# WithSecureOpenSource/async

Measured on AMD Instinct MI355X. Metric: GiB/s base64 encode+decode, device-resident, at 1/2/4/8 MI355X, higher is better.
Workload: dtype u8; 1 GPU; cfg2: one 1 GiB buffer per GPU, encode (std alphabet, pad) then decode, device-resident; bytes_per_gpu=1073741824, chars_per_gpu=1431655768, parallelism=independent buffers x1 (no data-path collective)

## Files before the change

### async_amd/_lib.py

```python
from __future__ import annotations

import ctypes
import errno
import os
import threading

_HERE = os.path.dirname(os.path.abspath(__file__))
LIB_PATH = os.path.join(_HERE, "libasync_b64.so")

_lock = threading.Lock()
_lib = None


class B64xError(RuntimeError):

    def __init__(self, func: str, code: int):
        self.code = code
        name = errno.errorcode.get(-code, str(code))
        super().__init__(f"{func} failed: {name} ({code})")


class Alphabet(ctypes.Structure):

    _fields_ = [
# ... 48 lines not shown
    "b64x_session_host_out": (_vp, [_vp]),
    "b64x_session_encode": (_int, [_vp, _u64, _ap, ctypes.POINTER(_u64)]),
    "b64x_release_stream": (None, [_vp]),
    "b64x_session_decode": (_int, [_vp, _u64, _ap, ctypes.c_uint, ctypes.POINTER(DecResult)]),
    "b64x_session_encode_async": (_int, [_vp, _u64, _ap, _vp, _vp]),
    "b64x_session_decode_async": (_int, [_vp, _u64, _ap, ctypes.c_uint, _vp, _vp]),
    "b64x_session_result": (ctypes.POINTER(DecResult), [_vp]),
    "b64x_session_decode_result": (_int, [_vp, ctypes.POINTER(DecResult)]),
    "b64x_session_wait": (_int, [_vp]),
    "b64x_host_alloc": (_vp, [_u64]),
    "b64x_host_free": (None, [_vp]),
    "b64x_lane_open": (_vp, []),
    "b64x_lane_close": (None, [_vp]),
    "b64x_lane_acquire": (_vp, []),
    "b64x_lane_release": (None, [_vp]),
    "b64x_lane_encode_async": (_int, [_vp, _vp, _u32, _vp, _vp, _vp, _vp, _u32, _ap, _vp, _vp]),
    "b64x_lane_encode_check": (_int, [_vp]),
    "b64x_lane_decode_async": (_int, [_vp, _vp, _u32, _vp, _vp, _vp, _vp, _vp, _vp, _vp, _ap,
                                      _vp, _vp, ctypes.POINTER(_u32)]),
    "b64x_lane_decode_check": (_int, [_vp, _u32, _vp, _vp, _vp, _vp, _vp, _u32]),
    "b64x_lane_wait": (_int, [_vp]),
    "b64x_diag_counters": (None, [ctypes.POINTER(_u64)]),
    "b64x_diag_paths": (None, [ctypes.POINTER(_u64)]),
    "b64x_fill_splitmix64": (_int, [_vp, _u64, _u64, _vp]),
    "b64x_device_check": (_int, []),
    "b64x_device_numa_node": (_int, [_int]),
    "b64x_bind_thread": (_int, [_int]),
    "b64x_build_info": (ctypes.c_char_p, []),
    "b64x_strerror": (ctypes.c_char_p, [_int]),
}

STAGE_SYMBOLS = [
    "base64_encode", "base64encoder_as_bytestream_1", "base64encoder_read",
    "base64encoder_close", "base64encoder_register_callback",
    "base64encoder_unregister_callback",
    "base64_decode", "base64decoder_as_bytestream_1", "base64decoder_read",
    "base64decoder_close", "base64decoder_register_callback",
    "base64decoder_unregister_callback",
    "make_async", "destroy_async", "async_now", "async_timer_start",
    "async_timer_cancel", "async_execute", "async_wound", "async_loop",
    "async_quit_loop", "async_register", "async_unregister",
    "NULL_ACTION_1", "bytestream_1_close_relaxed",
    "open_blobstream", "copy_blobstream", "adopt_blobstream",
    "blobstream_as_bytestream_1", "blobstream_remaining", "blobstream_read",
    "blobstream_close", "blobstream_register_callback",
    "blobstream_unregister_callback",
    "make_nice", "nicestream_as_bytestream_1", "nicestream_read",
    "nicestream_close", "nicestream_register_callback",
    "nicestream_unregister_callback",
]


def _import_torch_first() -> None:
    try:
        import torch
    except ImportError:
        pass


_DIAG_ONLY = {"b64x_diag_paths"}


def load() -> ctypes.CDLL:
    global _lib
    with _lock:
        if _lib is not None:
            return _lib
        if not os.path.exists(LIB_PATH):
            raise RuntimeError(
                f"{LIB_PATH} is missing: build it with `make` or "
                "__graft_entry__.build(); there is no CPU fallback")
        _import_torch_first()
        lib = ctypes.CDLL(LIB_PATH)
        for name, (res, args) in SIGNATURES.items():
            if name in _DIAG_ONLY and not hasattr(lib, name):
                continue
            fn = getattr(lib, name)
            fn.restype = res
            fn.argtypes = args
        _lib = lib
        return lib


# ... 18 lines not shown
```

### async_amd/csrc/b64x_kernels.hip

```cpp
#include <hip/hip_runtime.h>

#include <errno.h>
#include <sched.h>
#include <stdint.h>
#include <stdio.h>
#include <stdlib.h>
#include <string.h>
#include <sys/syscall.h>
#include <unistd.h>

#include <atomic>
#include <mutex>
#include <type_traits>
#include <utility>

#include "b64x.h"
#include "b64x_result_check.h"

#define DEV __device__ __forceinline__

namespace {

constexpr int kThreads = 256;
constexpr int kWavesPerBlock = kThreads / 64;
// ... 1395 lines not shown
    const uint32_t t2 = tab[(x >> 16) & 0xFFu], t3 = tab[x >> 24];
    const uint32_t lo = __builtin_amdgcn_perm(t1, t0, 0x0c0c0400u);
    const uint32_t hi = __builtin_amdgcn_perm(t3, t2, 0x0c0c0400u);
    return __builtin_amdgcn_perm(hi, lo, 0x05040100u);
}

constexpr uint32_t kProbeThreads = 256;

struct DecodeHint {
    uint32_t key, junky;
};
constexpr uint32_t kDecodeHints = 64;
constexpr uint64_t kProbeSampleMin = 1u << 18;
constexpr uint32_t kProbeNS = 256;
constexpr uint64_t kProbeTailKeep = 4096;

struct ProbeSmem {
    uint8_t tab[256];
    LineModel m;
    unsigned long long first;
};

DEV void probe_stream(ProbeSmem &ps, const uint8_t *__restrict__ in, uint64_t n, DecAlpha a,
                      void *ws, uint32_t nranges, DecodeHint *hint, uint32_t key, uint32_t publish)
{
    uint8_t *const tab = ps.tab;
    LineModel &s_m = ps.m;
    unsigned long long &s_first = ps.first;
    const bool sample = n >= kProbeSampleMin && threadIdx.x < kProbeNS;
    uint32_t sw[16];
    uint64_t q = 0;
    if (sample) {
        const uint64_t W = n - kProbeTailKeep - 64 - 256;
        const uint64_t span = threadIdx.x < kProbeNS / 2 ? W / 16 : W;
        const uint64_t i = threadIdx.x % (kProbeNS / 2) + 1;
        const uint64_t raw = 256 + span * i * i / ((uint64_t) kProbeNS * kProbeNS / 4);
        const uint8_t *pa = (const uint8_t *) ((uintptr_t) (in + raw) & ~(uintptr_t) 15);
        q = (uint64_t) (pa - in);
#pragma unroll
        for (uint32_t k = 0; k < 4; k++) {
            const uint4 x = *(const uint4 *) (pa + 16 * k);
            sw[4 * k] = x.x;
            sw[4 * k + 1] = x.y;
            sw[4 * k + 2] = x.z;
            sw[4 * k + 3] = x.w;
        }
    }
// ... 33 lines not shown
            const bool want = m.L == 0 || r < m.L;
            if (al != want && first == ~0ull) first = q + j;
            if (m.L && ++r == m.P) r = 0;
        }
        if (first != ~0ull) atomicMin(&s_first, (unsigned long long) first);
    }
    block_sync();
    if (threadIdx.x != 0) return;
    LineModel mo = m;
    const uint64_t pf = s_first;
    if (!mo.skip && pf != ~0ull) {
        const uint64_t F = mo.L ? pf / mo.P * mo.L + (pf % mo.P < mo.L ? pf % mo.P : mo.L) : pf;
        if (F / 16 < mo.T) {
            mo.T = (uint32_t) (F / 16);
            mo.skip = 1;
        }
    }
    if (mo.skip && publish) {
        *ws_view(ws, nranges).lfail = ~(uint64_t) mo.T;
        *ws_view(ws, nranges).fail_any = 1;
    }
    *ws_view(ws, nranges).model = mo;
    *ws_view(ws, nranges).model_n = n;
    if (hint) {
        volatile DecodeHint *h = hint;
        h->junky = mo.skip && 256 * (uint64_t) mo.T < n ? 1u : 0u;
        h->key = key;
    }
}

__global__ void __launch_bounds__(kProbeThreads) k_decode_probe(const uint8_t *__restrict__ in, uint64_t n,
                                                                DecAlpha a, void *ws, uint32_t nranges,
                                                                DecodeHint *hint, uint32_t key)
{
    __shared__ ProbeSmem ps;
    probe_stream(ps, in, n, a, ws, nranges, hint, key, 1u);
}

constexpr uint32_t kLinesTH = 256, kLinesWaves = kLinesTH / 64;

DEV void lines_first_fail(uint32_t badm, uint32_t &fail_u, uint32_t &fail_lane)
{
    if (__ballot(badm != 0) == 0) return;
#pragma unroll
    for (uint32_t u = 0; u < kLinesU; u++) {
        const uint64_t fb = __ballot((badm >> u) & 1u);
        if (fb) {
            fail_u = u;
            fail_lane = (uint32_t) __ffsll((unsigned long long) fb) - 1;
            return;
        }
    }
}

template <bool A4>
DEV uint32_t lines_hot(const uint8_t *tab, const uint8_t *__restrict__ inw, uint32_t pos0,
                       uint8_t *__restrict__ outw, uint32_t obase, const LineModel &m,
                       uint32_t col0, uint32_t lane)
{
// ... 13 lines not shown
        oo[u] = pos & 3u;
        const uint8_t *ab = inw + (pos & ~3u);
        win[u] = ld16<false>(ab);
        const u32x2a4 v = *(const u32x2a4 *) (ab + 16);
        wx[u] = make_uint2(v.x, v.y);
    }
    const uint32_t need = sep_need(s);
    uint32_t badm = 0;
#pragma unroll
    for (uint32_t u = 0; u < kLinesU; u++) {
        const uint32_t w6[6] = {win[u].x, win[u].y, win[u].z, win[u].w, wx[u].x, wx[u].y};
        uint32_t sep, G[4], bad;
        const uint4 d = A4 ? slot_chars4(w6, oo[u], cc[u] >> 2, s, &sep)
                           : slot_chars(w6, oo[u], cc[u], s, &sep);
        map_fast(tab, d, 16, G, bad);
        const uint32_t nd = hs[u] ? need : 0u;
        if ((sep_nonalpha(tab, sep) & nd) != nd) bad |= 0x100u;
        badm |= bad ? 1u << u : 0u;
        emit_full_off<true>(G, outw, obase + 12 * (u * 64 + lane));
    }
    return badm;
}

template <bool BIG>
__global__ __launch_bounds__(kLinesTH) __attribute__((amdgpu_waves_per_eu(6)))
void k_decode_lines(
    const uint8_t *__restrict__ in, uint64_t n, uint8_t *__restrict__ out, uint32_t nranges,
    DecAlpha a, void *ws, uint32_t hold, b64x_dec_result *res, uint32_t seq)
{
    __shared__ uint8_t tab[256];
    __shared__ uint8_t s_tail[64];
    const uint64_t *mp = (const uint64_t *) ws_view(ws, nranges).model;
    const uint64_t mw0 = scalar_load_u64(mp), mw1 = scalar_load_u64(mp + 1),
                   mw2 = scalar_load_u64(mp + 2), mw3 = scalar_load_u64(mp + 3);
    const uint64_t mn = scalar_load_u64(ws_view(ws, nranges).model_n);
    build_dec_table(tab, a);
    const bool mok = mn == n;
    const uint32_t T = mok ? (uint32_t) (mw1 >> 32) : (uint32_t) (n / 16);
    if (blockIdx.x * kLinesWaves * kLinesSlots > T) return;
    block_sync();
    LineModel m;
    m.L = mok ? (uint32_t) mw0 : 0u;
    m.s = (uint32_t) (mw0 >> 32);
    m.P = (uint32_t) mw1;
    m.T = T;
    m.m = (uint32_t) mw2;
    m.k = (uint32_t) (mw2 >> 32);
    m.rcp = (uint32_t) mw3;
    m.skip = mok ? (uint32_t) (mw3 >> 32) : 0u;
    const uint32_t lane = lane_id();
    const uint32_t L = m.L, s = m.s, P = m.P;
    const uint32_t wv = (uint32_t) __builtin_amdgcn_readfirstlane((int) (threadIdx.x >> 6));
    const uint32_t t0 = (blockIdx.x * kLinesWaves + wv) * kLinesSlots;
    if (t0 > T) return;
    const uint32_t ns = T - t0 >= kLinesSlots ? kLinesSlots : T - t0;
    const bool full = ns == kLinesSlots;
    const bool oal = (((uintptr_t) out) & 3) == 0;
    const bool ial = (((uintptr_t) in) & 3) == 0;
    uint32_t fail_u = kLinesU, fail_lane = 0;
    const uint64_t i0 = 16ull * t0;
    const uint32_t line0 = !L ? 0u : !BIG ? line_div(m, (uint32_t) i0) : (uint32_t) (i0 / L);
    const uint32_t col0 = (uint32_t) (i0 - (uint64_t) line0 * L);
    const uint64_t ie = i0 + 16 * ns;
    const uint32_t le = !L ? 0u : !BIG ? line_div(m, (uint32_t) ie) : (uint32_t) (ie / L);
    const bool safe = (L ? (uint64_t) le * P + (ie - (uint64_t) le * L) : ie) + 24 <= n;
    const uint64_t pos0 = (uint64_t) line0 * P;
    uint8_t *const outw = BIG ? out + 12ull * t0 : out;
    const uint32_t obase = BIG ? 0u : 12 * t0;
    if (ns && L == 0 && full && oal && ial) {
        uint4 c[kLinesU];
        const uint8_t *const inw = BIG ? in + 16ull * t0 : in;
        const uint32_t ibase = BIG ? 0u : 16 * t0;
#pragma unroll
        for (uint32_t u = 0; u < kLinesU; u++) c[u] = ld16<true>(inw + (ibase + 16 * (u * 64 + lane)));
        uint32_t badm = 0;
#pragma unroll
        for (uint32_t u = 0; u < kLinesU; u++) {
            uint32_t G[4], bad;
            map_fast(tab, c[u], 16, G, bad);
            badm |= bad ? 1u << u : 0u;
            emit_full_off<true>(G, outw, obase + 12 * (u * 64 + lane));
        }
        lines_first_fail(badm, fail_u, fail_lane);
    } else if (ns && L != 0 && full && oal && ial && safe) {
        const uint8_t *const inw = BIG ? in + (pos0 & ~3ull) : in;
        const uint32_t p0 = (uint32_t) (BIG ? pos0 & 3u : pos0);
        const uint32_t badm = (L & 3) == 0
            ? lines_hot<true>(tab, inw, p0, outw, obase, m, col0, lane)
            : lines_hot<false>(tab, inw, p0, outw, obase, m, col0, lane);
        lines_first_fail(badm, fail_u, fail_lane);
    } else if (ns) {
        uint32_t G[kLinesU][4], bad[kLinesU];
        const uint8_t *end = in + n;
        uint4 win[kLinesU];
        uint2 wx[kLinesU];
        uint32_t oo[kLinesU], cc[kLinesU];
        bool hs[kLinesU];
#pragma unroll
        for (uint32_t u = 0; u < kLinesU; u++) {
            const uint32_t rel = col0 + 16 * (u * 64 + lane);
            const uint32_t dl = L ? (rel * m.rcp) >> 20 : 0;
            const uint32_t col = rel - dl * L;
            const uint64_t pos = L ? (uint64_t) (line0 + dl) * P + col : i0 + 16 * (u * 64 + lane);
            hs[u] = L && L - col <= 16;
            cc[u] = hs[u] ? L - col : 16u;
            const uint8_t *ap = in + pos;
            const uint8_t *ab = (const uint8_t *) ((uintptr_t) ap & ~(uintptr_t) 3);
            oo[u] = (uint32_t) (ap - ab);
            const bool live = u * 64 + lane < ns;
            win[u] = live ? load_win16(ab, end) : make_uint4(0, 0, 0, 0);
            wx[u] = live ? load_win8(ab + 16, end) : make_uint2(0, 0);
        }
#pragma unroll
        for (uint32_t u = 0; u < kLinesU; u++) {
            const uint32_t w6[6] = {win[u].x, win[u].y, win[u].z, win[u].w, wx[u].x, wx[u].y};
            uint32_t sep;
            const uint4 d = slot_chars(w6, oo[u], cc[u], s, &sep);
            map_fast(tab, d, 16, G[u], bad[u]);
            const uint32_t need = sep_need(s);
            if (hs[u] && (sep_nonalpha(tab, sep) & need) != need) bad[u] |= 0x100u;
        }
#pragma unroll
        for (uint32_t u = 0; u < kLinesU; u++) {
            const bool live = u * 64 + lane < ns;
            const uint64_t fb = __ballot(live && bad[u] != 0);
            if (fb && fail_u == kLinesU) {
                fail_u = u;
                fail_lane = (uint32_t) __ffsll((unsigned long long) fb) - 1;
            }
            if (live) {
                uint32_t o0, o1, o2;
                groups_to_bytes(G[u][0], G[u][1], G[u][2], G[u][3], o0, o1, o2);
                store_bytes12(out + 12 * (uint64_t) (t0 + u * 64 + lane), o0, o1, o2, 12);
            }
        }
    }
    const bool cut = m.skip && T < t0 + kLinesSlots;
    if ((fail_u < kLinesU || cut) && lane == 0) {
        const unsigned long long key =
            ~(unsigned long long) (fail_u < kLinesU ? t0 + fail_u * 64 + fail_lane : T);
        unsigned long long *lf = (unsigned long long *) ws_view(ws, nranges).lfail +
                                 (blockIdx.x % kFailWords) * kFailStride;
        const unsigned long long cur =
            __hip_atomic_load(lf, __ATOMIC_RELAXED, __HIP_MEMORY_SCOPE_AGENT);
        if (key > cur) atomicMax(lf, key);
        if (cur == 0) *ws_view(ws, nranges).fail_any = 1;
    }
    if (T >= t0 + kLinesSlots || m.skip) return;
    const uint64_t Q = line_pos(m, 16 * (uint64_t) T);
    const uint32_t tl = (uint32_t) (n - Q);
    const bool here = lane < tl;
    const uint32_t tv = here ? tab[in[Q + lane]] : 0xFFu;
    const bool al = tv < 64u;
    const uint64_t mb = __ballot(al);
    const uint32_t Vt = (uint32_t) __popcll(mb);
    const uint32_t rank = __builtin_amdgcn_mbcnt_hi((uint32_t) (mb >> 32),
                                                    __builtin_amdgcn_mbcnt_lo((uint32_t) mb, 0u));
    if (al) s_tail[rank] = (uint8_t) tv;
    wave_lds_order();
// ... 3 lines not shown
        const uint32_t G = ((uint32_t) s_tail[4 * lane] << 18) | ((uint32_t) s_tail[4 * lane + 1] << 12) |
                           ((uint32_t) s_tail[4 * lane + 2] << 6) | s_tail[4 * lane + 3];
        ot[3 * lane] = (uint8_t) (G >> 16);
        ot[3 * lane + 1] = (uint8_t) (G >> 8);
        ot[3 * lane + 2] = (uint8_t) G;
    } else if (lane == ng && !hold && rem >= 2) {
        const uint32_t G = ((uint32_t) s_tail[4 * ng] << 18) | ((uint32_t) s_tail[4 * ng + 1] << 12) |
                           (rem > 2 ? (uint32_t) s_tail[4 * ng + 2] << 6 : 0u);
        ot[3 * ng] = (uint8_t) (G >> 16);
        if (rem > 2) ot[3 * ng + 1] = (uint8_t) (G >> 8);
    }
    if (lane == 0) {
        const uint64_t V = 16 * (uint64_t) T + Vt;
        b64x_dec_result r;
        r.out_len = hold ? V / 4 * 3 : V * 6 / 8;
        r.valid = V;
        r.tail_n = rem;
        for (uint32_t j = 0; j < 4; j++) r.tail[j] = j < rem ? s_tail[4 * ng + j] : 0;
        r.nchars = n;
        r.seq = seq;
        r.flags = hold ? 1u : 0u;
        *res = r;
    }
}

DEV void decode_range(const P2dSmem &sm, uint4 *bq, const uint8_t *__restrict__ in, uint64_t n,
                      uint64_t start, uint64_t re, int T0, uint8_t *ob, const uint4 c[2],
                      const uint32_t nin[2], uint32_t la, bool la_ok, bool last, uint32_t hold,
                      const uint8_t *la_lds = nullptr, bool la_late = false)
{
    const uint32_t lane = lane_id();
    uint32_t *bits = (uint32_t *) bq;
    int T = T0;
    const uint32_t skew = (uint32_t) ((uintptr_t) ob & 15);
    uint32_t lo = 16 + skew;
    int pb0 = 8 * (int) lo;
    uint32_t done = 0;
    static_assert(kP2dBlocks > 64 && kP2dBlocks <= 128, "two zeroing stores per lane");
    bq[lane] = make_uint4(0, 0, 0, 0);
    if (lane + 64 < kP2dBlocks) bq[lane + 64] = make_uint4(0, 0, 0, 0);
    wave_lds_order();
    T += (int) bits_step<true>(sm, bits, c, nin, pb0 + 6 * T);
    for (uint64_t pos = start + 2 * kChunk; pos < re; pos += 2 * kChunk) {
        wave_lds_order();
        const int bit_end = pb0 + 6 * T;
        const uint32_t kcut = bit_end > 0 ? ((uint32_t) bit_end >> 3) & ~15u : 0u;
// ... 131 lines not shown
        uint64_t B = scalar_load_u64(w.bases + r);
        while (r < mid_end) {
            const uint32_t rn = r + nw < mid_end ? r + nw : r;
            uint4 cn[2];
            cn[0] = load16_a4(in + (uint64_t) rn * R + 16 * lane);
            cn[1] = load16_a4(in + (uint64_t) rn * R + kChunk + 16 * lane);
            const uint32_t lan = ld_la(rn);
            const uint64_t Bn = scalar_load_u64(w.bases + rn);
            const uint64_t rb = (uint64_t) r * R;
            decode_range(sm, bq, in, n, rb, rb + R, range_skip(B), out + (B + 3) / 4 * 3, c, full,
                         la, (uint64_t) (r + 1) * R + lane < n, false, hold);
            r += nw;
            c[0] = cn[0];
            c[1] = cn[1];
            la = lan;
            B = Bn;
        }
    }
    for (; r < nranges; r += nw) generic(r);
}


DEV bool suffix_start(DecodeWs w, uint64_t n, b64x_dec_result *res, b64x_dec_result *hres,
                      uint64_t &S, uint64_t &Vb, uint32_t *reprobe)
{
    __shared__ uint64_t s_key;
    uint64_t key = 0;
    if (scalar_load_u64(w.fail_any) != 0) {
        if (threadIdx.x < 64) {
            key = __hip_atomic_load((unsigned long long *) w.lfail + (threadIdx.x % kFailWords) *
                                    kFailStride, __ATOMIC_RELAXED, __HIP_MEMORY_SCOPE_AGENT);
#pragma unroll
            for (int d = 32; d >= 1; d >>= 1) {
                const uint64_t o = __shfl_xor(key, d, 64);
                key = o > key ? o : key;
            }
        }
        if (threadIdx.x == 0) s_key = key;
        block_sync();
        key = s_key;
    }
    if (key == 0) {
        if (blockIdx.x == 0 && threadIdx.x == 0) {
            if (hres) {
                const b64x_dec_result r = *res;
                *hres = r;
            }
            *w.sfx_start = ~0ull;
        }
        return false;
    }
    Vb = 16 * ~key;
    S = scalar_load_u64(w.model_n) == n ? line_pos(*w.model, Vb) : Vb;
    if (reprobe && blockIdx.x == 0 && threadIdx.x == 0) *(volatile uint32_t *) reprobe = 1u;
    return true;
}


DEV uint32_t window_delta(uint32_t s, const uint8_t *dst)
{
    const uint32_t a = (uint32_t) ((uintptr_t) dst & 15);
    const uint32_t i0 = (s + (a ? 128u : 0u) - 8 * a) >> 5;
    return (4u - (i0 & 3u)) & 3u;
}

typedef uint32_t v4u32 __attribute__((ext_vector_type(4)));
typedef __attribute__((address_space(3))) const v4u32 lds_v4u32;

DEV void store_window_bits(const uint32_t *win, uint32_t s, uint32_t nb, uint8_t *dst)
{
    const uint32_t lane = lane_id();
    s = (uint32_t) __builtin_amdgcn_readfirstlane((int) s);
    nb = (uint32_t) __builtin_amdgcn_readfirstlane((int) nb);
    const uint32_t a = (uint32_t) ((uintptr_t) dst & 15);
    const uint32_t m0 = a ? 1u : 0u, mend = (nb + a) >> 4;
    const uint32_t b0 = s + 128 * m0 - 8 * a;
// ... 14 lines not shown
        const v4u32 g4 = __builtin_nontemporal_load((const lds_v4u32 *) (win + i));
        const uint4 g = make_uint4(g4.x, g4.y, g4.z, g4.w);
        const uint32_t w4 = win[i + 4];
        uint32_t o0 = g.x, o1 = g.y, o2 = g.z, o3 = g.w;
        if (sh) {
            const uint32_t r = 32u - sh;
            o0 = __builtin_amdgcn_alignbit(g.x, g.y, r);
            o1 = __builtin_amdgcn_alignbit(g.y, g.z, r);
            o2 = __builtin_amdgcn_alignbit(g.z, g.w, r);
            o3 = __builtin_amdgcn_alignbit(g.w, w4, r);
        }
        if (k < nblk)
            __builtin_nontemporal_store(u32x4a16{bswap32(o0), bswap32(o1), bswap32(o2), bswap32(o3)},
                                        (u32x4a16 *) (base + 16 * k));
    }
    if (act) dst[bi] = (uint8_t) ((((uint64_t) x0 << 32) | x1) >> (56 - (X & 31)));
}

template <bool WHOLE, bool BIG>
__global__ __launch_bounds__(kThreads) __attribute__((amdgpu_waves_per_eu(kHeldWaves)))
void k_decode_suffix_held(
    const uint8_t *__restrict__ in, uint64_t n, uint8_t *__restrict__ out, uint32_t nranges,
    DecAlpha a, void *ws, uint32_t hold, b64x_dec_result *res, b64x_dec_result *hres,
    uint32_t seq, uint32_t *reprobe, DecodeHint *hint, uint32_t key)
{
    constexpr uint64_t R = 2 * kChunk;
    constexpr uint32_t HP = kHeldPer, TILE = kHeldTile;
    DecodeWs w = ws_view(ws, nranges);
    uint64_t S = 0, Vb = 0;
    if (!WHOLE && !suffix_start(w, n, res, hres, S, Vb, reprobe)) return;
    uint8_t *base_out = out + Vb / 4 * 3;
    const uint32_t r0 = (uint32_t) (S / R);
    const uint32_t ntiles = (nranges - r0 + TILE - 1) / TILE;
    if (!WHOLE && blockIdx.x == 0 && threadIdx.x == 0) *w.sfx_start = S;
    const bool dma = (((uintptr_t) in) & 15) == 0;
    __shared__ P2dSmem sm;
    __shared__ uint4 s_rng[kWavesPerBlock][2][128];
    __shared__ uint32_t s_tile[2];
    using Cnt = typename std::conditional<BIG, uint64_t, uint32_t>::type;
    __shared__ uint32_t s_cnt[2][TILE];
    __shared__ Cnt s_excl;
    build_dec_table_lo(sm.tab, a);
    build_compact_sel<true>(sm.sel);
    const uint32_t lane = lane_id();
    const uint32_t wv = __builtin_amdgcn_readfirstlane(threadIdx.x >> 6);
    uint4 *bq = sm.bits[wv];
    uint32_t *bits = (uint32_t *) bq;

    auto publish = [&](uint32_t t, uint32_t b) {
        uint32_t agg = 0;
        for (uint32_t i = 0; i < TILE; i++) agg += s_cnt[b][i];
        st_store(&w.fstatus[t], kStAgg | agg);
        __hip_atomic_fetch_add(&w.fsuper[t / kSfxGroup], (1ull << 56) | agg, __ATOMIC_RELAXED,
// ... 179 lines not shown
                }
            }
            if (tA == ntiles - 1) {
                owner = true;
                Vs = exw;
                for (uint32_t i = 0; i < TILE; i++) Vs += s_cnt[bA][i];
            }
        }
        if (!haveB) break;
        LA = LB;
#pragma unroll
        for (uint32_t j = 0; j < HP; j++) {
#pragma unroll
            for (int i = 0; i < 6; i++) HA[j][i] = HB[j][i];
        }
        haveA = true;
        tA = tB;
        bA = bB;
        bB ^= 1u;
        if (threadIdx.x == 0) s_tile[bB] = atomicAdd(w.fticket, 1u);
    }
    if (WHOLE && hint && s_tile[bB] == ntiles) {
        __shared__ ProbeSmem ps;
        probe_stream(ps, in, n, a, ws, nranges, hint, key, 0u);
    }
    block_sync();
    if (threadIdx.x == 0) __hip_atomic_fetch_add(w.wdone, 1u, __ATOMIC_RELAXED, __HIP_MEMORY_SCOPE_AGENT);
    if (!owner || wv != 0) return;
    const uint64_t V = Vb + Vs;
    if (lane == 0) write_result(res, hres, V, hold, n, seq);
    find_tail_sextets<true>(sm.tab, in, n, V, res, hres);
    if (lane == 0) {
        while (__hip_atomic_load(w.wdone, __ATOMIC_RELAXED, __HIP_MEMORY_SCOPE_AGENT) != gridDim.x)
            __builtin_amdgcn_s_sleep(1);
    }
    for (uint32_t i = lane; i < ntiles; i += 64) st_store(&w.fstatus[i], 0);
    for (uint32_t i = lane; i < (ntiles + kSfxGroup - 1) / kSfxGroup; i += 64) st_store(&w.fsuper[i], 0);
    if (lane == 0) {
        __hip_atomic_store(w.fticket, 0u, __ATOMIC_RELAXED, __HIP_MEMORY_SCOPE_AGENT);
        __hip_atomic_store(w.wdone, 0u, __ATOMIC_RELAXED, __HIP_MEMORY_SCOPE_AGENT);
        for (uint32_t i = 0; i < kFailWords; i++) w.lfail[i * kFailStride] = 0;
        *w.fail_any = 0;
    }
}

struct BatchLayout {
    const uint64_t *in_off;
// ... 1379 lines not shown

struct HeldModel {
    const void *ws;
    uint64_t n;
};
constexpr int kHeldModels = 64;
std::mutex g_held_mu;
HeldModel g_held[kHeldModels];

static uint32_t *held_reprobe(int slot)
{
    static uint32_t *h = nullptr;
    static std::once_flag once;
    std::call_once(once, [] {
        void *p = nullptr;
        if (hipHostMalloc(&p, kHeldModels * 64, hipHostMallocCoherent) == hipSuccess) {
            memset(p, 0, kHeldModels * 64);
            h = (uint32_t *) p;
        }
    });
    return h ? h + 16 * slot : nullptr;
}

static int held_slot(const void *ws)
{
    const uint64_t x = (uintptr_t) ws * 0x9E3779B97F4A7C15ull;
    return (int) (x >> 58);
}

enum { kPathProbe, kPathHeld, kPathHinted, kPathRowsPrep, kPathRowsReuse, kPaths };
static std::atomic<uint64_t> g_paths[kPaths];

static void path_taken(int k) { g_paths[k].fetch_add(1, std::memory_order_relaxed); }

void b64x_diag_paths(uint64_t out[5])
{
    for (int k = 0; k < kPaths; k++) out[k] = g_paths[k].load(std::memory_order_relaxed);
}

static uint32_t hint_key(const void *ws, const void *in, uint64_t n)
{
    uint64_t x = (uintptr_t) ws * 0x9E3779B97F4A7C15ull ^ (uintptr_t) in * 0xC2B2AE3D27D4EB4Full ^
                 n * 0x165667B19E3779F9ull;
    x ^= x >> 31;
    return (uint32_t) (x >> 32) | 1u;
}


static int decode_dev_ws(const void *d_in, uint64_t nchars, void *d_out,
                         b64x_dec_result *d_res, b64x_dec_result *h_res,
                         const b64x_alphabet *abc, unsigned flags, void *ws, void *stream,
                         uint32_t seq, const DeviceInfo *d)
{
    hipStream_t s = (hipStream_t) stream;
    int err = 0;
    const RangePlan p = plan_ranges(nchars);
    const uint32_t blocks = (p.nranges + kWavesPerBlock - 1) / kWavesPerBlock;
    const DecAlpha a = dec_alpha(abc);
    const uint32_t hold = flags & B64X_DEC_HOLD_TAIL;
    if (p.R == 2 * kChunk) {
        const bool big = nchars > (1ull << 31);
        static const int occ_small = occupancy_of(k_decode_suffix_held<false, false>);
        static const int occ_big = occupancy_of(k_decode_suffix_held<false, true>);
        const int occ_sfx = big ? occ_big : occ_small;
        auto *const k_whole = big ? k_decode_suffix_held<true, true> : k_decode_suffix_held<true, false>;
        auto *const k_sfx = big ? k_decode_suffix_held<false, true> : k_decode_suffix_held<false, false>;
        auto *const k_lines = big ? k_decode_lines<true> : k_decode_lines<false>;
        const uint32_t sfx_grid = (uint32_t) d->cus * occ_sfx;
        if (flags & B64X_DEC_EXPECT_JUNK) {
            hipLaunchKernelGGL(k_whole, dim3(sfx_grid), dim3(kThreads), 0, s,
                               (const uint8_t *) d_in, nchars, (uint8_t *) d_out, p.nranges, a, ws,
                               hold, d_res, h_res, seq, nullptr, nullptr, 0u);
            return launch_status();
        }
        DecodeHint *hints = decode_hints();
        const uint32_t key = hint_key(ws, d_in, nchars);
        DecodeHint *hint = hints ? hints + (key % kDecodeHints) : nullptr;
        const bool junky = hint && ((volatile DecodeHint *) hint)->key == key &&
                           ((volatile DecodeHint *) hint)->junky;
        const int hs = held_slot(ws);
        uint32_t *reprobe = held_reprobe(hs);
        bool reuse = false;
        if (!junky && reprobe && !capturing(stream)) {
            std::lock_guard<std::mutex> lk(g_held_mu);
            reuse = g_held[hs].ws == ws && g_held[hs].n == nchars &&
                    !*(volatile uint32_t *) reprobe;
        }
        if (junky) {
            path_taken(kPathHinted);
            if (reprobe) *(volatile uint32_t *) reprobe = 0;
            hipLaunchKernelGGL(k_whole, dim3(sfx_grid), dim3(kThreads), 0, s,
                               (const uint8_t *) d_in, nchars, (uint8_t *) d_out, p.nranges, a, ws,
                               hold, d_res, h_res, seq, nullptr, hint, key);
            if ((err = launch_status())) return err;
            path_taken(kPathProbe);
            std::lock_guard<std::mutex> lk(g_held_mu);
            g_held[hs] = HeldModel{ws, nchars};
            return 0;
        }
        if (!reuse) {
            if (reprobe) *(volatile uint32_t *) reprobe = 0;
            hipLaunchKernelGGL(k_decode_probe, dim3(1), dim3(kProbeThreads), 0, s,
                               (const uint8_t *) d_in, nchars, a, ws, p.nranges, hint, key);
            if ((err = launch_status())) return err;
            path_taken(kPathProbe);
            std::lock_guard<std::mutex> lk(g_held_mu);
            g_held[hs] = HeldModel{ws, nchars};
        } else {
            path_taken(kPathHeld);
        }
        const uint64_t waves = (nchars / 16 + 1 + kLinesSlots - 1) / kLinesSlots;
        hipLaunchKernelGGL(k_lines, dim3((uint32_t) ((waves + kLinesWaves - 1) / kLinesWaves)),
                           dim3(kLinesTH), 0, s, (const uint8_t *) d_in, nchars, (uint8_t *) d_out,
                           p.nranges, a, ws, hold, d_res, seq);
        if ((err = launch_status())) return err;
        hipLaunchKernelGGL(k_sfx, dim3(sfx_grid), dim3(kThreads), 0, s,
                           (const uint8_t *) d_in, nchars, (uint8_t *) d_out, p.nranges, a, ws,
                           hold, d_res, h_res, seq, reprobe, nullptr, 0u);
        return launch_status();
    }
    hipLaunchKernelGGL(k_pass1, dim3(blocks), dim3(kThreads), 0, s, (const uint8_t *) d_in,
                       nchars, (uint8_t *) d_out, p.R, p.nranges, a, ws, hold);
    if ((err = launch_status())) return err;
    hipLaunchKernelGGL(k_decode_scan2, dim3((p.nranges + kScanTile - 1) / kScanTile),
                       dim3(kThreads), 0, s, (const uint8_t *) d_in, nchars, p.R, p.nranges, a,
                       ws, d_res, h_res, hold, seq);
    if ((err = launch_status())) return err;
    static const int occ2d = occupancy_of(k_decode_pass2d);
    const uint32_t b2 = cap_grid(blocks, (uint64_t) d->cus * occ2d);
    hipLaunchKernelGGL(k_decode_pass2d, dim3(b2), dim3(kThreads), 0, s,
                       (const uint8_t *) d_in, nchars, (uint8_t *) d_out, p.R, p.nranges,
                       a, ws, hold);
    return launch_status();
}

static int decode_dev_impl(const void *d_in, uint64_t nchars, void *d_out,
                           b64x_dec_result *d_res, b64x_dec_result *h_res,
                           const b64x_alphabet *abc, unsigned flags, void *d_workspace,
                           void *stream, uint32_t seq)
{
    if (!d_res) return -EINVAL;
// ... 928 lines not shown
```

### include/b64x.h

```cpp

#ifndef ASYNC_AMD_B64X_H
#define ASYNC_AMD_B64X_H

#include <stdbool.h>
#include <stddef.h>
#include <stdint.h>

#ifdef __cplusplus
extern "C" {
#endif

#define B64X_ABI_VERSION 4

typedef struct b64x_alphabet {
    char pos62;
    char pos63;
    char padchar;
    bool pad;
} b64x_alphabet;

typedef struct b64x_dec_result {
    uint64_t out_len;
    uint64_t valid;
    uint32_t tail_n;
// ... 87 lines not shown
    const uint8_t *src;
} b64x_seg;
int b64x_lane_encode_async(b64x_lane *l, const uint8_t *h_in, uint32_t njobs,
                           const uint64_t *h_in_off, uint8_t *h_out,
                           const uint64_t *h_out_off, const b64x_seg *h_seg, uint32_t nseg,
                           const b64x_alphabet *abc, b64x_done_fn done, void *arg);
int b64x_lane_encode_check(b64x_lane *l);
#define B64X_LANE_CHAINED 4u

int b64x_lane_decode_async(b64x_lane *l, const uint8_t *h_in, uint32_t njobs,
                           const uint64_t *h_in_off, uint8_t *h_out,
                           const uint64_t *h_out_off, const uint8_t *h_flags,
                           b64x_dec_result *h_res, const b64x_dec_result *const *h_prev,
                           b64x_dec_result *h_spell, const b64x_alphabet *abc,
                           b64x_done_fn done, void *arg, uint32_t *seq);
int b64x_lane_decode_check(b64x_lane *l, uint32_t seq, const uint64_t *h_in_off,
                           const uint8_t *h_flags, const b64x_dec_result *h_res,
                           const b64x_dec_result *const *h_prev,
                           const b64x_dec_result *h_spell, uint32_t njobs);
int b64x_lane_wait(b64x_lane *l);

void b64x_diag_counters(uint64_t out[2]);
void b64x_diag_paths(uint64_t out[5]);


int b64x_fill_splitmix64(void *d_out, uint64_t n, uint64_t seed,
                         void *stream);

int b64x_device_check(void);


int b64x_device_numa_node(int device);
int b64x_bind_thread(int device);
const char *b64x_build_info(void);
const char *b64x_strerror(int err);

#ifdef __cplusplus
}
#endif

#endif
```

Before: 1287 GiB/s.

## Add clean-input fast path to decode-lines kernel skipping model loads

The probe kernel now records whether the stream has no line breaks or junk, and the host caches that flag per workspace. On reuse with a clean, aligned, non-big buffer, k_decode_lines takes a specialized path: it issues the input loads before building the decode table, builds the table with one entry per thread, and skips reading the line model from the workspace. The suffix kernel skips the line_pos mapping for clean inputs. The intent is to shorten the decode kernel's startup latency, at the cost of relying on cached state from an earlier probe being valid for the same buffer.

```diff
diff --git a/async_amd/_lib.py b/async_amd/_lib.py
--- a/async_amd/_lib.py
+++ b/async_amd/_lib.py
@@ -94,6 +94,7 @@
     "b64x_lane_wait": (_int, [_vp]),
     "b64x_diag_counters": (None, [ctypes.POINTER(_u64)]),
     "b64x_diag_paths": (None, [ctypes.POINTER(_u64)]),
+    "b64x_diag_clean_launches": (_u64, []),
     "b64x_fill_splitmix64": (_int, [_vp, _u64, _u64, _vp]),
     "b64x_device_check": (_int, []),
     "b64x_device_numa_node": (_int, [_int]),
@@ -130,7 +131,7 @@
         pass
 
 
-_DIAG_ONLY = {"b64x_diag_paths"}
+_DIAG_ONLY = {"b64x_diag_paths", "b64x_diag_clean_launches"}
 
 
 def load() -> ctypes.CDLL:
diff --git a/async_amd/csrc/b64x_kernels.hip b/async_amd/csrc/b64x_kernels.hip
--- a/async_amd/csrc/b64x_kernels.hip
+++ b/async_amd/csrc/b64x_kernels.hip
@@ -1441,7 +1441,8 @@
 };
 
 DEV void probe_stream(ProbeSmem &ps, const uint8_t *__restrict__ in, uint64_t n, DecAlpha a,
-                      void *ws, uint32_t nranges, DecodeHint *hint, uint32_t key, uint32_t publish)
+                      void *ws, uint32_t nranges, DecodeHint *hint, uint32_t key, uint32_t publish,
+                      uint64_t *clean_n)
 {
     uint8_t *const tab = ps.tab;
     LineModel &s_m = ps.m;
@@ -1521,6 +1522,7 @@
     }
     *ws_view(ws, nranges).model = mo;
     *ws_view(ws, nranges).model_n = n;
+    if (clean_n) *(volatile uint64_t *) clean_n = mo.L == 0 && !mo.skip ? n : 0ull;
     if (hint) {
         volatile DecodeHint *h = hint;
         h->junky = mo.skip && 256 * (uint64_t) mo.T < n ? 1u : 0u;
@@ -1530,10 +1532,11 @@
 
 __global__ void __launch_bounds__(kProbeThreads) k_decode_probe(const uint8_t *__restrict__ in, uint64_t n,
                                                                 DecAlpha a, void *ws, uint32_t nranges,
-                                                                DecodeHint *hint, uint32_t key)
+                                                                DecodeHint *hint, uint32_t key,
+                                                                uint64_t *clean_n)
 {
     __shared__ ProbeSmem ps;
-    probe_stream(ps, in, n, a, ws, nranges, hint, key, 1u);
+    probe_stream(ps, in, n, a, ws, nranges, hint, key, 1u, clean_n);
 }
 
 constexpr uint32_t kLinesTH = 256, kLinesWaves = kLinesTH / 64;
@@ -1593,119 +1596,64 @@
     return badm;
 }
 
-template <bool BIG>
-__global__ __launch_bounds__(kLinesTH) __attribute__((amdgpu_waves_per_eu(6)))
-void k_decode_lines(
-    const uint8_t *__restrict__ in, uint64_t n, uint8_t *__restrict__ out, uint32_t nranges,
-    DecAlpha a, void *ws, uint32_t hold, b64x_dec_result *res, uint32_t seq)
-{
-    __shared__ uint8_t tab[256];
-    __shared__ uint8_t s_tail[64];
-    const uint64_t *mp = (const uint64_t *) ws_view(ws, nranges).model;
-    const uint64_t mw0 = scalar_load_u64(mp), mw1 = scalar_load_u64(mp + 1),
-                   mw2 = scalar_load_u64(mp + 2), mw3 = scalar_load_u64(mp + 3);
-    const uint64_t mn = scalar_load_u64(ws_view(ws, nranges).model_n);
-    build_dec_table(tab, a);
-    const bool mok = mn == n;
-    const uint32_t T = mok ? (uint32_t) (mw1 >> 32) : (uint32_t) (n / 16);
-    if (blockIdx.x * kLinesWaves * kLinesSlots > T) return;
-    block_sync();
-    LineModel m;
-    m.L = mok ? (uint32_t) mw0 : 0u;
-    m.s = (uint32_t) (mw0 >> 32);
-    m.P = (uint32_t) mw1;
-    m.T = T;
-    m.m = (uint32_t) mw2;
-    m.k = (uint32_t) (mw2 >> 32);
-    m.rcp = (uint32_t) mw3;
-    m.skip = mok ? (uint32_t) (mw3 >> 32) : 0u;
-    const uint32_t lane = lane_id();
+DEV void lines_guarded(const uint8_t *tab, const uint8_t *__restrict__ in, uint64_t n,
+                       uint8_t *__restrict__ out, const LineModel &m, uint32_t t0, uint32_t ns,
+                       uint32_t line0, uint32_t col0, uint64_t i0, uint32_t lane,
+                       uint32_t &fail_u, uint32_t &fail_lane)
+{
     const uint32_t L = m.L, s = m.s, P = m.P;
-    const uint32_t wv = (uint32_t) __builtin_amdgcn_readfirstlane((int) (threadIdx.x >> 6));
-    const uint32_t t0 = (blockIdx.x * kLinesWaves + wv) * kLinesSlots;
-    if (t0 > T) return;
-    const uint32_t ns = T - t0 >= kLinesSlots ? kLinesSlots : T - t0;
-    const bool full = ns == kLinesSlots;
-    const bool oal = (((uintptr_t) out) & 3) == 0;
-    const bool ial = (((uintptr_t) in) & 3) == 0;
-    uint32_t fail_u = kLinesU, fail_lane = 0;
-    const uint64_t i0 = 16ull * t0;
-    const uint32_t line0 = !L ? 0u : !BIG ? line_div(m, (uint32_t) i0) : (uint32_t) (i0 / L);
-    const uint32_t col0 = (uint32_t) (i0 - (uint64_t) line0 * L);
-    const uint64_t ie = i0 + 16 * ns;
-    const uint32_t le = !L ? 0u : !BIG ? line_div(m, (uint32_t) ie) : (uint32_t) (ie / L);
-    const bool safe = (L ? (uint64_t) le * P + (ie - (uint64_t) le * L) : ie) + 24 <= n;
-    const uint64_t pos0 = (uint64_t) line0 * P;
-    uint8_t *const outw = BIG ? out + 12ull * t0 : out;
-    const uint32_t obase = BIG ? 0u : 12 * t0;
-    if (ns && L == 0 && full && oal && ial) {
-        uint4 c[kLinesU];
-        const uint8_t *const inw = BIG ? in + 16ull * t0 : in;
-        const uint32_t ibase = BIG ? 0u : 16 * t0;
-#pragma unroll
-        for (uint32_t u = 0; u < kLinesU; u++) c[u] = ld16<true>(inw + (ibase + 16 * (u * 64 + lane)));
-        uint32_t badm = 0;
-#pragma unroll
-        for (uint32_t u = 0; u < kLinesU; u++) {
-            uint32_t G[4], bad;
-            map_fast(tab, c[u], 16, G, bad);
-            badm |= bad ? 1u << u : 0u;
-            emit_full_off<true>(G, outw, obase + 12 * (u * 64 + lane));
-        }
-        lines_first_fail(badm, fail_u, fail_lane);
-    } else if (ns && L != 0 && full && oal && ial && safe) {
-        const uint8_t *const inw = BIG ? in + (pos0 & ~3ull) : in;
-        const uint32_t p0 = (uint32_t) (BIG ? pos0 & 3u : pos0);
-        const uint32_t badm = (L & 3) == 0
-            ? lines_hot<true>(tab, inw, p0, outw, obase, m, col0, lane)
-            : lines_hot<false>(tab, inw, p0, outw, obase, m, col0, lane);
-        lines_first_fail(badm, fail_u, fail_lane);
-    } else if (ns) {
-        uint32_t G[kLinesU][4], bad[kLinesU];
-        const uint8_t *end = in + n;
-        uint4 win[kLinesU];
-        uint2 wx[kLinesU];
-        uint32_t oo[kLinesU], cc[kLinesU];
-        bool hs[kLinesU];
-#pragma unroll
-        for (uint32_t u = 0; u < kLinesU; u++) {
-            const uint32_t rel = col0 + 16 * (u * 64 + lane);
-            const uint32_t dl = L ? (rel * m.rcp) >> 20 : 0;
-            const uint32_t col = rel - dl * L;
-            const uint64_t pos = L ? (uint64_t) (line0 + dl) * P + col : i0 + 16 * (u * 64 + lane);
-            hs[u] = L && L - col <= 16;
-            cc[u] = hs[u] ? L - col : 16u;
-            const uint8_t *ap = in + pos;
-            const uint8_t *ab = (const uint8_t *) ((uintptr_t) ap & ~(uintptr_t) 3);
-            oo[u] = (uint32_t) (ap - ab);
-            const bool live = u * 64 + lane < ns;
-            win[u] = live ? load_win16(ab, end) : make_uint4(0, 0, 0, 0);
-            wx[u] = live ? load_win8(ab + 16, end) : make_uint2(0, 0);
-        }
-#pragma unroll
-        for (uint32_t u = 0; u < kLinesU; u++) {
-            const uint32_t w6[6] = {win[u].x, win[u].y, win[u].z, win[u].w, wx[u].x, wx[u].y};
-            uint32_t sep;
-            const uint4 d = slot_chars(w6, oo[u], cc[u], s, &sep);
-            map_fast(tab, d, 16, G[u], bad[u]);
-            const uint32_t need = sep_need(s);
-            if (hs[u] && (sep_nonalpha(tab, sep) & need) != need) bad[u] |= 0x100u;
-        }
-#pragma unroll
-        for (uint32_t u = 0; u < kLinesU; u++) {
-            const bool live = u * 64 + lane < ns;
-            const uint64_t fb = __ballot(live && bad[u] != 0);
-            if (fb && fail_u == kLinesU) {
-                fail_u = u;
-                fail_lane = (uint32_t) __ffsll((unsigned long long) fb) - 1;
-            }
-            if (live) {
-                uint32_t o0, o1, o2;
-                groups_to_bytes(G[u][0], G[u][1], G[u][2], G[u][3], o0, o1, o2);
-                store_bytes12(out + 12 * (uint64_t) (t0 + u * 64 + lane), o0, o1, o2, 12);
-            }
-        }
-    }
+    uint32_t G[kLinesU][4], bad[kLinesU];
+    const uint8_t *end = in + n;
+    uint4 win[kLinesU];
+    uint2 wx[kLinesU];
+    uint32_t oo[kLinesU], cc[kLinesU];
+    bool hs[kLinesU];
+#pragma unroll
+    for (uint32_t u = 0; u < kLinesU; u++) {
+        const uint32_t rel = col0 + 16 * (u * 64 + lane);
+        const uint32_t dl = L ? (rel * m.rcp) >> 20 : 0;
+        const uint32_t col = rel - dl * L;
+        const uint64_t pos = L ? (uint64_t) (line0 + dl) * P + col : i0 + 16 * (u * 64 + lane);
+        hs[u] = L && L - col <= 16;
+        cc[u] = hs[u] ? L - col : 16u;
+        const uint8_t *ap = in + pos;
+        const uint8_t *ab = (const uint8_t *) ((uintptr_t) ap & ~(uintptr_t) 3);
+        oo[u] = (uint32_t) (ap - ab);
+        const bool live = u * 64 + lane < ns;
+        win[u] = live ? load_win16(ab, end) : make_uint4(0, 0, 0, 0);
+        wx[u] = live ? load_win8(ab + 16, end) : make_uint2(0, 0);
+    }
+#pragma unroll
+    for (uint32_t u = 0; u < kLinesU; u++) {
+        const uint32_t w6[6] = {win[u].x, win[u].y, win[u].z, win[u].w, wx[u].x, wx[u].y};
+        uint32_t sep;
+        const uint4 d = slot_chars(w6, oo[u], cc[u], s, &sep);
+        map_fast(tab, d, 16, G[u], bad[u]);
+        const uint32_t need = sep_need(s);
+        if (hs[u] && (sep_nonalpha(tab, sep) & need) != need) bad[u] |= 0x100u;
+    }
+#pragma unroll
+    for (uint32_t u = 0; u < kLinesU; u++) {
+        const bool live = u * 64 + lane < ns;
+        const uint64_t fb = __ballot(live && bad[u] != 0);
+        if (fb && fail_u == kLinesU) {
+            fail_u = u;
+            fail_lane = (uint32_t) __ffsll((unsigned long long) fb) - 1;
+        }
+        if (live) {
+            uint32_t o0, o1, o2;
+            groups_to_bytes(G[u][0], G[u][1], G[u][2], G[u][3], o0, o1, o2);
+            store_bytes12(out + 12 * (uint64_t) (t0 + u * 64 + lane), o0, o1, o2, 12);
+        }
+    }
+}
+
+DEV void lines_finish(const uint8_t *tab, uint8_t *s_tail, const uint8_t *__restrict__ in,
+                      uint64_t n, uint8_t *__restrict__ out, const LineModel &m, uint32_t t0,
+                      void *ws, uint32_t nranges, uint32_t hold, b64x_dec_result *res, uint32_t seq,
+                      uint32_t lane, uint32_t fail_u, uint32_t fail_lane)
+{
+    const uint32_t T = m.T;
     const bool cut = m.skip && T < t0 + kLinesSlots;
     if ((fail_u < kLinesU || cut) && lane == 0) {
         const unsigned long long key =
@@ -1755,6 +1703,125 @@
         r.flags = hold ? 1u : 0u;
         *res = r;
     }
+}
+
+DEV void lines_clean(uint8_t *tab, uint8_t *s_tail, const uint8_t *__restrict__ in, uint64_t n,
+                     uint8_t *__restrict__ out, DecAlpha a, void *ws, uint32_t nranges,
+                     uint32_t hold, b64x_dec_result *res, uint32_t seq)
+{
+    LineModel m{};
+    m.T = (uint32_t) (n / 16);
+    const uint32_t wv = (uint32_t) __builtin_amdgcn_readfirstlane((int) (threadIdx.x >> 6));
+    const uint32_t t0 = (blockIdx.x * kLinesWaves + wv) * kLinesSlots;
+    const bool full = t0 + kLinesSlots <= m.T;
+    uint4 c[kLinesU];
+    if (full) {
+        uint32_t ll = threadIdx.x;
+        asm volatile("" : "+v"(ll));
+        ll &= 63u;
+#pragma unroll
+        for (uint32_t u = 0; u < kLinesU; u++) c[u] = ld16<true>(in + (16 * t0 + 16 * (u * 64 + ll)));
+    }
+    static_assert(kLinesTH == 256, "one table entry per thread");
+    tab[threadIdx.x] = (uint8_t) dec_value(threadIdx.x, a);
+    block_sync();
+    if (t0 > m.T) return;
+    const uint32_t lane = lane_id();
+    uint32_t fail_u = kLinesU, fail_lane = 0;
+    if (full) {
+        uint32_t badm = 0;
+#pragma unroll
+        for (uint32_t u = 0; u < kLinesU; u++) {
+            uint32_t G[4], bad;
+            map_fast(tab, c[u], 16, G, bad);
+            badm |= bad ? 1u << u : 0u;
+            emit_full_off<true>(G, out, 12 * t0 + 12 * (u * 64 + lane));
+        }
+        lines_first_fail(badm, fail_u, fail_lane);
+    } else if (m.T - t0) {
+        lines_guarded(tab, in, n, out, m, t0, m.T - t0, 0u, 0u, 16ull * t0, lane, fail_u, fail_lane);
+    }
+    lines_finish(tab, s_tail, in, n, out, m, t0, ws, nranges, hold, res, seq, lane, fail_u, fail_lane);
+}
+
+template <bool BIG>
+__global__ __launch_bounds__(kLinesTH) __attribute__((amdgpu_waves_per_eu(6)))
+void k_decode_lines(
+    const uint8_t *__restrict__ in, uint64_t n, uint8_t *__restrict__ out, uint32_t nranges,
+    uint32_t clean, int p62, int p63, void *ws, uint32_t hold, b64x_dec_result *res, uint32_t seq)
+{
+    __shared__ uint8_t tab[256];
+    __shared__ uint8_t s_tail[64];
+    const DecAlpha a{p62, p63};
+    if constexpr (!BIG) {
+        if (clean) {
+            lines_clean(tab, s_tail, in, n, out, a, ws, nranges, hold, res, seq);
+            return;
+        }
+    }
+    const uint64_t *mp = (const uint64_t *) ws_view(ws, nranges).model;
+    const uint64_t mw0 = scalar_load_u64(mp), mw1 = scalar_load_u64(mp + 1),
+                   mw2 = scalar_load_u64(mp + 2), mw3 = scalar_load_u64(mp + 3);
+    const uint64_t mn = scalar_load_u64(ws_view(ws, nranges).model_n);
+    build_dec_table(tab, a);
+    const bool mok = mn == n;
+    const uint32_t T = mok ? (uint32_t) (mw1 >> 32) : (uint32_t) (n / 16);
+    if (blockIdx.x * kLinesWaves * kLinesSlots > T) return;
+    block_sync();
+    LineModel m;
+    m.L = mok ? (uint32_t) mw0 : 0u;
+    m.s = (uint32_t) (mw0 >> 32);
+    m.P = (uint32_t) mw1;
+    m.T = T;
+    m.m = (uint32_t) mw2;
+    m.k = (uint32_t) (mw2 >> 32);
+    m.rcp = (uint32_t) mw3;
+    m.skip = mok ? (uint32_t) (mw3 >> 32) : 0u;
+    const uint32_t lane = lane_id();
+    const uint32_t L = m.L, P = m.P;
+    const uint32_t wv = (uint32_t) __builtin_amdgcn_readfirstlane((int) (threadIdx.x >> 6));
+    const uint32_t t0 = (blockIdx.x * kLinesWaves + wv) * kLinesSlots;
+    if (t0 > T) return;
+    const uint32_t ns = T - t0 >= kLinesSlots ? kLinesSlots : T - t0;
+    const bool full = ns == kLinesSlots;
+    const bool oal = (((uintptr_t) out) & 3) == 0;
+    const bool ial = (((uintptr_t) in) & 3) == 0;
+    uint32_t fail_u = kLinesU, fail_lane = 0;
+    const uint64_t i0 = 16ull * t0;
+    const uint32_t line0 = !L ? 0u : !BIG ? line_div(m, (uint32_t) i0) : (uint32_t) (i0 / L);
+    const uint32_t col0 = (uint32_t) (i0 - (uint64_t) line0 * L);
+    const uint64_t ie = i0 + 16 * ns;
+    const uint32_t le = !L ? 0u : !BIG ? line_div(m, (uint32_t) ie) : (uint32_t) (ie / L);
+    const bool safe = (L ? (uint64_t) le * P + (ie - (uint64_t) le * L) : ie) + 24 <= n;
+    const uint64_t pos0 = (uint64_t) line0 * P;
+    uint8_t *const outw = BIG ? out + 12ull * t0 : out;
+    const uint32_t obase = BIG ? 0u : 12 * t0;
+    if (ns && L == 0 && full && oal && ial) {
+        uint4 c[kLinesU];
+        const uint8_t *const inw = BIG ? in + 16ull * t0 : in;
+        const uint32_t ibase = BIG ? 0u : 16 * t0;
+#pragma unroll
+        for (uint32_t u = 0; u < kLinesU; u++) c[u] = ld16<true>(inw + (ibase + 16 * (u * 64 + lane)));
+        uint32_t badm = 0;
+#pragma unroll
+        for (uint32_t u = 0; u < kLinesU; u++) {
+            uint32_t G[4], bad;
+            map_fast(tab, c[u], 16, G, bad);
+            badm |= bad ? 1u << u : 0u;
+            emit_full_off<true>(G, outw, obase + 12 * (u * 64 + lane));
+        }
+        lines_first_fail(badm, fail_u, fail_lane);
+    } else if (ns && L != 0 && full && oal && ial && safe) {
+        const uint8_t *const inw = BIG ? in + (pos0 & ~3ull) : in;
+        const uint32_t p0 = (uint32_t) (BIG ? pos0 & 3u : pos0);
+        const uint32_t badm = (L & 3) == 0
+            ? lines_hot<true>(tab, inw, p0, outw, obase, m, col0, lane)
+            : lines_hot<false>(tab, inw, p0, outw, obase, m, col0, lane);
+        lines_first_fail(badm, fail_u, fail_lane);
+    } else if (ns) {
+        lines_guarded(tab, in, n, out, m, t0, ns, line0, col0, i0, lane, fail_u, fail_lane);
+    }
+    lines_finish(tab, s_tail, in, n, out, m, t0, ws, nranges, hold, res, seq, lane, fail_u, fail_lane);
 }
 
 DEV void decode_range(const P2dSmem &sm, uint4 *bq, const uint8_t *__restrict__ in, uint64_t n,
@@ -1932,7 +1999,7 @@
 
 
 DEV bool suffix_start(DecodeWs w, uint64_t n, b64x_dec_result *res, b64x_dec_result *hres,
-                      uint64_t &S, uint64_t &Vb, uint32_t *reprobe)
+                      uint64_t &S, uint64_t &Vb, uint32_t *reprobe, uint32_t clean)
 {
     __shared__ uint64_t s_key;
     uint64_t key = 0;
@@ -1961,7 +2028,7 @@
         return false;
     }
     Vb = 16 * ~key;
-    S = scalar_load_u64(w.model_n) == n ? line_pos(*w.model, Vb) : Vb;
+    S = !clean && scalar_load_u64(w.model_n) == n ? line_pos(*w.model, Vb) : Vb;
     if (reprobe && blockIdx.x == 0 && threadIdx.x == 0) *(volatile uint32_t *) reprobe = 1u;
     return true;
 }
@@ -2022,13 +2089,14 @@
 void k_decode_suffix_held(
     const uint8_t *__restrict__ in, uint64_t n, uint8_t *__restrict__ out, uint32_t nranges,
     DecAlpha a, void *ws, uint32_t hold, b64x_dec_result *res, b64x_dec_result *hres,
-    uint32_t seq, uint32_t *reprobe, DecodeHint *hint, uint32_t key)
+    uint32_t seq, uint32_t *reprobe, DecodeHint *hint, uint32_t key, uint64_t *clean_n,
+    uint32_t clean)
 {
     constexpr uint64_t R = 2 * kChunk;
     constexpr uint32_t HP = kHeldPer, TILE = kHeldTile;
     DecodeWs w = ws_view(ws, nranges);
     uint64_t S = 0, Vb = 0;
-    if (!WHOLE && !suffix_start(w, n, res, hres, S, Vb, reprobe)) return;
+    if (!WHOLE && !suffix_start(w, n, res, hres, S, Vb, reprobe, clean)) return;
     uint8_t *base_out = out + Vb / 4 * 3;
     const uint32_t r0 = (uint32_t) (S / R);
     const uint32_t ntiles = (nranges - r0 + TILE - 1) / TILE;
@@ -2254,7 +2322,7 @@
     }
     if (WHOLE && hint && s_tile[bB] == ntiles) {
         __shared__ ProbeSmem ps;
-        probe_stream(ps, in, n, a, ws, nranges, hint, key, 0u);
+        probe_stream(ps, in, n, a, ws, nranges, hint, key, 0u, clean_n);
     }
     block_sync();
     if (threadIdx.x == 0) __hip_atomic_fetch_add(w.wdone, 1u, __ATOMIC_RELAXED, __HIP_MEMORY_SCOPE_AGENT);
@@ -3680,6 +3748,11 @@
     return h ? h + 16 * slot : nullptr;
 }
 
+static uint64_t *held_clean_n(uint32_t *reprobe)
+{
+    return reprobe ? (uint64_t *) (reprobe + 2) : nullptr;
+}
+
 static int held_slot(const void *ws)
 {
     const uint64_t x = (uintptr_t) ws * 0x9E3779B97F4A7C15ull;
@@ -3694,6 +3767,13 @@
 void b64x_diag_paths(uint64_t out[5])
 {
     for (int k = 0; k < kPaths; k++) out[k] = g_paths[k].load(std::memory_order_relaxed);
+}
+
+static std::atomic<uint64_t> g_clean_launches;
+
+uint64_t b64x_diag_clean_launches(void)
+{
+    return g_clean_launches.load(std::memory_order_relaxed);
 }
 
 static uint32_t hint_key(const void *ws, const void *in, uint64_t n)
@@ -3728,7 +3808,7 @@
         if (flags & B64X_DEC_EXPECT_JUNK) {
             hipLaunchKernelGGL(k_whole, dim3(sfx_grid), dim3(kThreads), 0, s,
                                (const uint8_t *) d_in, nchars, (uint8_t *) d_out, p.nranges, a, ws,
-                               hold, d_res, h_res, seq, nullptr, nullptr, 0u);
+                               hold, d_res, h_res, seq, nullptr, nullptr, 0u, nullptr, 0u);
             return launch_status();
         }
         DecodeHint *hints = decode_hints();
@@ -3738,18 +3818,24 @@
                            ((volatile DecodeHint *) hint)->junky;
         const int hs = held_slot(ws);
         uint32_t *reprobe = held_reprobe(hs);
+        uint64_t *clean_n = held_clean_n(reprobe);
         bool reuse = false;
+        uint32_t clean = 0;
         if (!junky && reprobe && !capturing(stream)) {
             std::lock_guard<std::mutex> lk(g_held_mu);
             reuse = g_held[hs].ws == ws && g_held[hs].n == nchars &&
                     !*(volatile uint32_t *) reprobe;
+            clean = reuse && *(volatile uint64_t *) clean_n == nchars && !big &&
+                    nchars >= 16 * kLinesSlots &&
+                    ((((uintptr_t) d_in) | ((uintptr_t) d_out)) & 3) == 0;
         }
         if (junky) {
             path_taken(kPathHinted);
             if (reprobe) *(volatile uint32_t *) reprobe = 0;
+            if (clean_n) *(volatile uint64_t *) clean_n = 0;
             hipLaunchKernelGGL(k_whole, dim3(sfx_grid), dim3(kThreads), 0, s,
                                (const uint8_t *) d_in, nchars, (uint8_t *) d_out, p.nranges, a, ws,
-                               hold, d_res, h_res, seq, nullptr, hint, key);
+                               hold, d_res, h_res, seq, nullptr, hint, key, clean_n, 0u);
             if ((err = launch_status())) return err;
             path_taken(kPathProbe);
             std::lock_guard<std::mutex> lk(g_held_mu);
@@ -3758,23 +3844,25 @@
         }
         if (!reuse) {
             if (reprobe) *(volatile uint32_t *) reprobe = 0;
+            if (clean_n) *(volatile uint64_t *) clean_n = 0;
             hipLaunchKernelGGL(k_decode_probe, dim3(1), dim3(kProbeThreads), 0, s,
-                               (const uint8_t *) d_in, nchars, a, ws, p.nranges, hint, key);
+                               (const uint8_t *) d_in, nchars, a, ws, p.nranges, hint, key, clean_n);
             if ((err = launch_status())) return err;
             path_taken(kPathProbe);
             std::lock_guard<std::mutex> lk(g_held_mu);
             g_held[hs] = HeldModel{ws, nchars};
         } else {
             path_taken(kPathHeld);
+            if (clean) g_clean_launches.fetch_add(1, std::memory_order_relaxed);
         }
         const uint64_t waves = (nchars / 16 + 1 + kLinesSlots - 1) / kLinesSlots;
         hipLaunchKernelGGL(k_lines, dim3((uint32_t) ((waves + kLinesWaves - 1) / kLinesWaves)),
                            dim3(kLinesTH), 0, s, (const uint8_t *) d_in, nchars, (uint8_t *) d_out,
-                           p.nranges, a, ws, hold, d_res, seq);
+                           p.nranges, clean, a.p62, a.p63, ws, hold, d_res, seq);
         if ((err = launch_status())) return err;
         hipLaunchKernelGGL(k_sfx, dim3(sfx_grid), dim3(kThreads), 0, s,
                            (const uint8_t *) d_in, nchars, (uint8_t *) d_out, p.nranges, a, ws,
-                           hold, d_res, h_res, seq, reprobe, nullptr, 0u);
+                           hold, d_res, h_res, seq, reprobe, nullptr, 0u, nullptr, clean);
         return launch_status();
     }
     hipLaunchKernelGGL(k_pass1, dim3(blocks), dim3(kThreads), 0, s, (const uint8_t *) d_in,
diff --git a/include/b64x.h b/include/b64x.h
--- a/include/b64x.h
+++ b/include/b64x.h
@@ -133,6 +133,7 @@
 
 void b64x_diag_counters(uint64_t out[2]);
 void b64x_diag_paths(uint64_t out[5]);
+uint64_t b64x_diag_clean_launches(void);
 
 
 int b64x_fill_splitmix64(void *d_out, uint64_t n, uint64_t seed,
```

New measurement: 1287 GiB/s, median of 2. No clear change (-0.0%).
